# ArbiterMob/FluidSimulationCuda

Measured on AMD Instinct MI355X. Metric: Mcells/s per Jacobi iter, higher is better.
Workload: dtype f32

## Files before the change

### fluidsimulationcuda_amd/capi.py

```python
import ctypes as C
import os

import numpy as np

from ._build import LIB

OK, E_INVALID, E_NOMEM, E_HIP, E_COMM = 0, 1, 2, 3, 4
U, V, DENS, U_PREV, V_PREV, DENS_PREV, TMP0, TMP1, TMP2, TMP3, TMP4, TMP5 = range(12)
NFIELDS = 12
JACOBI_STREAM, JACOBI_LDS, JACOBI_NAIVE, JACOBI_TB = 0, 1, 2, 3
STORAGE_F32, STORAGE_F16 = 0, 1
PARAM_TB_MAX_SWEEPS, PARAM_TB_ROWS, PARAM_HALO, PARAM_TB_FAST_DIVISION, PARAM_TB_MIN_CELLS, PARAM_TB_EDGE_ROWS_PCT = 0, 1, 2, 3, 4, 5
PARAM_TB_LANE_COLUMNS = 6
PARAM_TB_T16_MIN_CELLS = 7
PARAM_TB_AUTOTUNE = 8
PARAM_FUSE_DIVERGENCE = 9
PARAM_SLAB_OVERLAP = 10
PARAM_EARLY_ADVECT = 11
PARAM_FUSE_ADD_SOURCE = 12
PARAM_XCHG_OVERLAP = 13
PARAM_F16_PRESSURE_SCALE = 14
PARAM_TB_FILL = 15
XCHG_HALO, XCHG_GATHER, XCHG_MAX, XCHG_MAX_BEGIN, XCHG_MAX_END = 0, 1, 2, 3, 4
RCCL_ID_BYTES = 128
FIELD_NAMES = ("u", "v", "dens", "u_prev", "v_prev", "dens_prev", "tmp0", "tmp1", "tmp2", "tmp3", "tmp4", "tmp5")


class FluidError(RuntimeError):
    def __init__(self, code, msg):
        super().__init__("libfluid_amd error %d: %s" % (code, msg))
        self.code = code


class Config(C.Structure):
    _fields_ = [("n", C.c_int), ("rank", C.c_int), ("nranks", C.c_int), ("halo", C.c_int),
                ("jacobi_variant", C.c_int), ("stream", C.c_void_p), ("arena", C.c_void_p),
                ("arena_bytes", C.c_size_t), ("storage", C.c_int)]


TIME_SOURCE, TIME_DIFFUSION, TIME_DIVERGENCE, TIME_PROJECTION, TIME_ADVECTION = range(5)
TIMING_CATEGORIES = ("source", "diffusion", "divergence", "projection", "advection")


class Timing(C.Structure):
    _fields_ = [("jacobi_ms", C.c_double), ("sweeps", C.c_longlong), ("solves", C.c_longlong),
# ... 133 lines not shown
```

### fluidsimulationcuda_amd/csrc/fluid_ctx.h

```cpp
#pragma once
#include <hip/hip_runtime.h>

#include <string>
#include <utility>
#include <vector>

#include "../../include/fluid_amd.h"
#include "fluid_kernels.h"

namespace fluid_detail {
int fail(int code, const char* fmt, ...);
int materialize_zero(fluid_ctx* c, int f);
int refuse_ensemble(const fluid_ctx* c, const char* what);
struct RcclExchange;
void rccl_release(RcclExchange* x);
}

#define HIP_TRY(expr)                                                                                      \
    do {                                                                                                   \
        hipError_t e_ = (expr);                                                                            \
        if (e_ != hipSuccess)                                                                              \
            return fluid_detail::fail(e_ == hipErrorOutOfMemory ? FLUID_E_NOMEM : FLUID_E_HIP, "%s: %s",   \
                                      #expr, hipGetErrorString(e_));                                       \
    } while (0)
// ... 88 lines not shown
    hipEvent_t ev_xbegin = nullptr, ev_xdone = nullptr;
    bool xchg_overlap = true;
    unsigned xowed = 0;
    long long split_launches = 0;
    bool early_advect = true;
    float vmax_prev[2] = {-1.0f, -1.0f};
    FieldState field[FLUID_NFIELDS];
    size_t field_bytes = 0;
    unsigned int* d_scalar = nullptr;
    float* d_partials = nullptr;
    ConstRing consts;
    EnsembleReduce red;
    MemberStage stage;
    TransformTables xform;
    unsigned int* tiles = nullptr;
    unsigned int* h_scalar = nullptr;
    hipEvent_t scalar_ready = nullptr;
    int variant = fluid::JACOBI_TB;
    int tb_max_t = 16, tb_rows = 0, num_cu = 256;
    long long tb_min_cells = 0;
    long long tb_t16_min_cells = -1;
    bool fuse_divergence = true;
    bool tb_fill = true;
    bool autotune = true;
    struct Trial { unsigned long long key; int cand; hipEvent_t a, b; };
    std::vector<Trial> trials;
    std::vector<hipEvent_t> free_events;
    bool defer_zero_source = true;
    bool in_halo_exchange = false;
    int tb_nv = 2;
    int tb_edge_pct = 40;
    int fast_div = 2;
    int rank = 0, nranks = 1, own0 = 1, own1 = 1, min_slab = 0, halo = 1;
    bool fuse_add_source = true;
    float pscale = 1.0f;
    fluid_exchange_fn xchg = nullptr;
    void* xchg_user = nullptr;
    fluid_detail::RcclExchange* rccl = nullptr;
    bool timing = false;
    struct Ev { hipEvent_t a, b; int cat; bool pressure; };
    std::vector<Ev> ev_pool;
    size_t ev_used = 0;
    double cat_ms[FLUID_TIMING_CATEGORIES] = {};
    long long cat_calls[FLUID_TIMING_CATEGORIES] = {};
    long long sweeps = 0, pending_sweeps = 0, launches = 0, field_launches = 0;
    double pressure_ms = 0.0;
// ... 13 lines not shown
```

### fluidsimulationcuda_amd/csrc/fluid_kernels.h

```cpp
#pragma once
#include <hip/hip_runtime.h>

namespace fluid {

constexpr int XOFF = 63;

enum JacobiVariant { JACOBI_STREAM = 0, JACOBI_LDS = 1, JACOBI_NAIVE = 2, JACOBI_TB = 3, JACOBI_VARIANTS = 4 };

enum Storage { STORAGE_F32 = 0, STORAGE_F16 = 1 };
typedef _Float16 half_t;
inline size_t storage_bytes(int st) { return st == STORAGE_F16 ? 2 : 4; }

inline int pitch_for(int n) { return ((XOFF + 1 + 4 * ((n + 3) / 4) + 1) + 63) / 64 * 64; }

struct Members {
    int count = 1;
    size_t stride = 0;
};

struct TbMemberK {
    double yd;
    float alpha, beta, hi, lo;
    float x0_inc, div_scale;
    unsigned tile_thr, pad;
};

struct TbBatch {
    const void* x[3];
    const void* x0[3];
    void* out[3];
    float alpha[3], beta[3];
    double yd[3];
    float hi[3], lo[3];
    const unsigned* tiles[3];
    unsigned tile_thr[3];
    int tile_pitch;
    void* div[3];
    float div_scale;
    int b[3];
    int x_zero[3];
    float x0_inc[3];
    int count;
    int members;
    size_t mstride;
    size_t tile_mstride;
    const TbMemberK* mk;
};

void launch_set_bnd(hipStream_t s, int st, void* f, int pitch, int n, int b, Members mb = {});
void launch_add_source(hipStream_t s, int st, void* x, const void* src, int pitch, int row_lo, int row_hi, float dt, Members mb = {},
                       const float* mdt = nullptr);
void launch_jacobi(hipStream_t s, int st, int variant, const void* x, const void* x0, void* out, int pitch, int n,
                   int row_lo, int row_hi, float alpha, float beta, int b, Members mb = {}, const float2* mab = nullptr);
enum TbForm { TB_PLAIN = 0, TB_DIVSRC = 1, TB_ADDSRC = 2 };
struct TbShape { int T, divmode, nv, form; };
inline constexpr TbShape kTbShapes[] = {
    {2, 0, 2, TB_PLAIN},   {2, 2, 2, TB_PLAIN},   {2, 3, 2, TB_PLAIN},   {2, 4, 2, TB_PLAIN},   {2, 5, 2, TB_PLAIN},
    {2, 0, 4, TB_PLAIN},   {2, 2, 4, TB_PLAIN},   {2, 3, 4, TB_PLAIN},   {2, 4, 4, TB_PLAIN},   {2, 5, 4, TB_PLAIN},
    {4, 0, 2, TB_PLAIN},   {4, 2, 2, TB_PLAIN},   {4, 3, 2, TB_PLAIN},   {4, 4, 2, TB_PLAIN},   {4, 5, 2, TB_PLAIN},
    {4, 0, 4, TB_PLAIN},   {4, 2, 4, TB_PLAIN},   {4, 3, 4, TB_PLAIN},   {4, 4, 4, TB_PLAIN},   {4, 5, 4, TB_PLAIN},
    {8, 0, 2, TB_PLAIN},   {8, 2, 2, TB_PLAIN},   {8, 3, 2, TB_PLAIN},   {8, 4, 2, TB_PLAIN},   {8, 5, 2, TB_PLAIN},
    {8, 0, 4, TB_PLAIN},   {8, 2, 4, TB_PLAIN},   {8, 3, 4, TB_PLAIN},   {8, 4, 4, TB_PLAIN},   {8, 5, 4, TB_PLAIN},
    {12, 0, 2, TB_PLAIN},  {12, 2, 2, TB_PLAIN},  {12, 3, 2, TB_PLAIN},  {12, 4, 2, TB_PLAIN},  {12, 5, 2, TB_PLAIN},
// ... 77 lines not shown
```

### fluidsimulationcuda_amd/csrc/fluid_kernels.hip

```cpp
#include <hip/hip_runtime.h>
#include <stdint.h>

#include <algorithm>
#include <array>
#include <cstdlib>
#include <utility>

#include "fluid_kernels.h"

namespace fluid {

__device__ __forceinline__ float flip_if(bool c, float v) { return c ? -v : v; }

__device__ __forceinline__ float keep_f32(float v) { asm("" : "+v"(v)); return v; }
__device__ __forceinline__ float ld1(const float* p) { return *p; }
__device__ __forceinline__ float ld1(const half_t* p) { return keep_f32((float)*p); }
__device__ __forceinline__ void st1(float* p, float v) { *p = v; }
__device__ __forceinline__ void st1(half_t* p, float v) { *p = (half_t)keep_f32(v); }
template <typename S>
__device__ __forceinline__ float as_stored(float v)
{
    if constexpr (sizeof(S) == 2) return keep_f32((float)(S)keep_f32(v));
    else return v;
}
// ... 376 lines not shown
constexpr float kDiv5NegScale = -0x1p24f;

template <typename S, int NV>
struct TbArgs {
    const S* xc;
    const S* rc;
    S* oc;
    __amdgpu_buffer_rsrc_t bx, br, bo;
    unsigned ld_off;
    unsigned st_off;
    unsigned row_bytes;
    unsigned m_lg;
    unsigned m_r[NV];
    int n, q_lo, q_hi, cg;
    float alpha;
    DivK k;
    S* dc;
    __amdgpu_buffer_rsrc_t bd;
    float div_scale;
    int s_lo, s_hi;
    unsigned sx, sy;
    float x0_inc;
    bool st_rg_lane, is_lg;
    bool fill;
};

__device__ __forceinline__ float fxor(float v, unsigned m) { return __uint_as_float(__float_as_uint(v) ^ m); }
template <int NV>
__device__ __forceinline__ Vec<NV> fxorv(const Vec<NV>& v, unsigned m)
{
    Vec<NV> o;
#pragma unroll
    for (int c = 0; c < NV; ++c) o.c[c] = fxor(v.c[c], m);
    return o;
}

template <int DIVMODE>
__device__ __forceinline__ float tb_div(float num, const DivK& k)
{
    if (DIVMODE == 0) return num / k.beta;
    if (DIVMODE == 4) return num * k.beta;
    if (DIVMODE == 3) return __builtin_fmaf(num, k.hi, num * k.lo);
    if (DIVMODE == 5) {
        const float q0 = num * k.beta;
        const float e = __builtin_fmaf(q0, k.hi, num * kDiv5NegScale);
        return __builtin_fmaf(e, k.lo, q0);
// ... 44 lines not shown
{
    unsigned long long n = 0;
    const unsigned long long stride = (unsigned long long)gridDim.x * 256;
    auto differs = [](float got, float ref) { return (ref != ref) ? !(got != got) : (__float_as_uint(got) != __float_as_uint(ref)); };
    DivK k2 = k;
    for (unsigned long long i = (unsigned long long)blockIdx.x * 256 + threadIdx.x; i < (1ull << 32); i += stride) {
        const float a = __uint_as_float((unsigned)i);
        const float ref = a / beta;
        if constexpr (DIVMODE == 3) {
            const bool in_range = a == 0.0f || !(__builtin_fabsf(a) < beta * 0x1p-98f);
            n += differs(tb_div<2>(a, k2), ref) || (in_range && differs(tb_div<3>(a, k), ref));
        } else if constexpr (DIVMODE == 5) {
            const float got = tb_div<5>(a, k);
            const bool finite = __builtin_fabsf(got) < __builtin_inff();
            const bool must_be_exact = __builtin_fabsf(a) < 0x1p100f;
            n += differs(got, ref) && (finite || must_be_exact);
        } else {
            n += differs(tb_div<DIVMODE>(a, k), ref);
        }
    }
    if (n) atomicAdd(bad, n);
}

__device__ __forceinline__ float bitsel(unsigned mask, float a, float b)
{
    return __uint_as_float((__float_as_uint(a) & mask) | (__float_as_uint(b) & ~mask));
}

template <typename S, int NV>
__device__ __forceinline__ void tb_fix_columns(Vec<NV>& G, const TbArgs<S, NV>& a, float& v1, float& vn, bool need_corners)
{
    float o[NV];
#pragma unroll
    for (int c = 0; c < NV; ++c) o[c] = G.c[c];
    const float from_right = lane_above0(o[0]);
    const float from_left = lane_below0(o[NV - 1]);
    G.c[0] = bitsel(a.m_r[0], fxor(from_left, a.sx), o[0]);
#pragma unroll
    for (int c = 1; c < NV - 1; ++c) G.c[c] = bitsel(a.m_r[c], fxor(o[c - 1], a.sx), o[c]);
    G.c[NV - 1] = bitsel(a.m_lg, fxor(from_right, a.sx), bitsel(a.m_r[NV - 1], fxor(o[NV - 2], a.sx), o[NV - 1]));
    if (need_corners) {
        v1 = from_right;
        unsigned bits = __float_as_uint(from_left) & a.m_r[0];
#pragma unroll
        for (int c = 1; c < NV; ++c) bits |= __float_as_uint(o[c - 1]) & a.m_r[c];
        vn = __uint_as_float(bits);
    }
}

template <bool EDGE, bool WALL, typename S, int NV>
__device__ __forceinline__ void tb_store_to(S* oc, __amdgpu_buffer_rsrc_t bo, const Vec<NV>& G, int q, bool mine, const TbArgs<S, NV>& a,
                                            float v1, float vn)
{
    auto on = [](bool c, unsigned off) { return c ? off : kBufOff; };
    buf_stv<NV>(oc, bo, on(mine, a.st_off) + (unsigned)q * a.row_bytes, G);
    if (WALL) {
        Vec<NV> g = fxorv<NV>(G, a.sy);
        if (EDGE) {
            const float cl = 0.5f * (fxor(v1, a.sy) + fxor(v1, a.sx));
            const float cr = 0.5f * (fxor(vn, a.sy) + fxor(vn, a.sx));
            if (a.is_lg) g.c[NV - 1] = cl;
#pragma unroll
            for (int c = 0; c < NV; ++c)
                if (a.st_rg_lane && a.cg == c) g.c[c] = cr;
        }
        buf_stv<NV>(oc, bo, on(mine & (q == 1), a.st_off), g);
        buf_stv<NV>(oc, bo, on(mine & (q == a.n), a.st_off) + (unsigned)(a.n + 1) * a.row_bytes, g);
    }
}
template <bool EDGE, bool WALL, typename S, int NV>
__device__ __forceinline__ void tb_store(const Vec<NV>& G, int q, bool mine, const TbArgs<S, NV>& a, float v1, float vn)
{
    tb_store_to<EDGE, WALL, S, NV>(a.oc, a.bo, G, q, mine, a, v1, vn);
}

template <int NV>
__device__ __forceinline__ Vec<NV> tb_divergence(const Vec<NV>& u, const Vec<NV>& v_up, const Vec<NV>& v_dn, float scale)
{
    float g[NV];
#pragma unroll
    for (int c = 0; c < NV; ++c) {
        const float ur = c < NV - 1 ? u.c[c + 1] : lane_above0(u.c[0]);
        const float ul = c > 0 ? u.c[c - 1] : lane_below0(u.c[NV - 1]);
        g[c] = ur - ul;
    }
    Vec<NV> d;
#pragma unroll
    for (int p = 0; p < NV; p += 2) {
        v2f s = {g[p], g[p + 1]};
        s = s + (v2f){v_dn.c[p], v_dn.c[p + 1]};
        s = s - (v2f){v_up.c[p], v_up.c[p + 1]};
        s = s * scale;
        d.c[p] = s.x;
// ... 14 lines not shown
        o.c[p + 1] = out.y;
    }
    return o;
}

template <int K, int N, int NV>
__device__ __forceinline__ void tb_qshift(Vec<NV> (&Q)[N])
{
    if constexpr (K >= 1) {
        Q[K] = Q[K - 1];
        tb_qshift<K - 1, N, NV>(Q);
    }
}

template <int DIVMODE, int NV>
__device__ __forceinline__ void tb_sticky(const Vec<NV>& G, v2f& nf)
{
    if constexpr (DIVMODE == 5) {
#pragma unroll
        for (int p = 0; p < NV; p += 2) nf = __builtin_elementwise_fma((v2f){G.c[p], G.c[p + 1]}, (v2f){0.f, 0.f}, nf);
    }
}

template <int T, int DIVMODE, bool EDGE, bool WALL, bool GEN, int PH, typename S, int NV, bool DIVSRC = false, bool ADDSRC = false,
          bool PART = false>
__device__ __forceinline__ void tb_step(int t, Vec<NV> (&W)[T][3], Vec<NV> (&Q)[T + 1], Vec<NV> (&PX)[3], Vec<NV> (&PQ)[3],
                                        const TbArgs<S, NV>& a, Vec<NV> (&UR)[3], Vec<NV> (&VR)[3], v2f& nf, int smax = T)
{
    static_assert(!(PART && GEN), "the general body runs every stage");
    constexpr int UP = PH % 3, ME = (PH + 1) % 3, FR = (PH + 2) % 3;
    __builtin_amdgcn_sched_barrier(0);
    if constexpr (DIVSRC) {
        UR[FR] = take<NV>(PX[PH]);
        VR[FR] = take<NV>(PQ[PH]);
    } else {
        W[0][FR] = take<NV>(PX[PH]);
        Q[0] = take<NV>(PQ[PH]);
        if constexpr (ADDSRC) {
#pragma unroll
            for (int p = 0; p < NV; p += 2) {
                const v2f ds = (v2f){W[0][FR].c[p], W[0][FR].c[p + 1]} * a.div_scale;
                const v2f q = (v2f){Q[0].c[p], Q[0].c[p + 1]} + ds;
                Q[0].c[p] = as_stored<S>(q.x);
                Q[0].c[p + 1] = as_stored<S>(q.y);
            }
            buf_stv<NV>(a.dc, a.bd, (((t >= a.s_lo) & (t < a.s_hi)) ? a.st_off : kBufOff) + (unsigned)t * a.row_bytes, Q[0]);
        } else {
#pragma unroll
            for (int p = 0; p < NV; p += 2) {
                const v2f q = (v2f){Q[0].c[p], Q[0].c[p + 1]} + a.x0_inc;
                Q[0].c[p] = q.x;
                Q[0].c[p + 1] = q.y;
            }
        }
    }
    {
        const unsigned off = a.ld_off + (unsigned)(t + 3) * a.row_bytes;
        PX[PH] = buf_ldv<NV>(a.xc, a.bx, off);
        PQ[PH] = buf_ldv<NV>(a.rc, a.br, off);
    }
    __builtin_amdgcn_sched_barrier(0);
    if constexpr (DIVSRC) {
        const int q = t - 1;
        Vec<NV> D = tb_divergence<NV>(UR[ME], VR[UP], VR[FR], a.div_scale);
#pragma unroll
        for (int c = 0; c < NV; ++c) D.c[c] = as_stored<S>(D.c[c]);
        Q[1] = D;
        float v1 = 0.f, vn = 0.f;
        if (EDGE) tb_fix_columns<S, NV>(D, a, v1, vn, WALL);
        tb_store_to<EDGE, (WALL || GEN), S, NV>(a.dc, a.bd, D, q, (q >= 1) & (q <= a.n) & (q >= a.q_lo) & (q < a.q_hi), a, v1, vn);
    }
    if constexpr (!GEN) {
#pragma unroll
        for (int s = 1; s <= T; ++s) {
            const bool run = !PART || s <= smax;
            const int q = t - s;
            Vec<NV> G;
            float v1 = 0.f, vn = 0.f;
            if (run) {
                G = tb_stencil<DIVMODE, NV>(W[s - 1][UP], W[s - 1][ME], W[s - 1][FR], Q[s], a.alpha, a.k);
                if (EDGE) tb_fix_columns<S, NV>(G, a, v1, vn, WALL && s == T);
                if (s == T) tb_sticky<DIVMODE, NV>(G, nf);
            } else {
#pragma unroll
                for (int c = 0; c < NV; ++c) G.c[c] = __builtin_nondeterministic_value(W[s - 1][FR].c[c]);
            }
            if (s < T) W[s][FR] = G;
            else tb_store<EDGE, WALL, S, NV>(G, q, run & (q >= a.q_lo) & (q < a.q_hi), a, v1, vn);
        }
    } else {
#pragma unroll
        for (int s = 1; s <= T; ++s) {
            const int q = t - s;
            const bool interior = (q >= 1 && q <= a.n);
            Vec<NV> G = tb_stencil<DIVMODE, NV>(W[s - 1][UP], W[s - 1][ME], W[s - 1][FR], Q[s], a.alpha, a.k);
            float v1 = 0.f, vn = 0.f;
            if (EDGE) tb_fix_columns<S, NV>(G, a, v1, vn, s == T);
            if (s < T) {
                const Vec<NV> me = W[s][ME];
                const Vec<NV> flipped_me = fxorv<NV>(me, a.sy);
                const Vec<NV> flipped_g = fxorv<NV>(G, a.sy);
                const bool bot_ghost = (q == a.n + 1), top_ghost = (q == 1);
#pragma unroll
                for (int c = 0; c < NV; ++c) {
                    W[s][FR].c[c] = bot_ghost ? flipped_me.c[c] : G.c[c];
                    W[s][ME].c[c] = top_ghost ? flipped_g.c[c] : me.c[c];
                }
            } else {
                tb_sticky<DIVMODE, NV>(G, nf);
                tb_store<EDGE, true, S, NV>(G, q, interior & (q >= a.q_lo) & (q < a.q_hi), a, v1, vn);
            }
        }
    }
    tb_qshift<T, T + 1, NV>(Q);
}

template <int T, int DIVMODE, bool EDGE, bool WALL, typename S, int NV, bool DIVSRC = false, bool ADDSRC = false>
__device__ __forceinline__ bool tb_march(int t0, int t1, const TbArgs<S, NV>& a)
{
    Vec<NV> W[T][3], Q[T + 1], PX[3], PQ[3], UR[3], VR[3];
    v2f nf = {0.f, 0.f};
    Vec<NV> zero;
#pragma unroll
    for (int c = 0; c < NV; ++c) zero.c[c] = 0.f;
#pragma unroll
    for (int s = 0; s < T; ++s) { W[s][0] = zero; W[s][1] = zero; W[s][2] = zero; }
#pragma unroll
    for (int s = 0; s <= T; ++s) Q[s] = zero;
#pragma unroll
    for (int d = 0; d < 3; ++d) { UR[d] = zero; VR[d] = zero; }
#pragma unroll
    for (int d = 0; d < 3; ++d) {
        const unsigned off = a.ld_off + (unsigned)(t0 + d) * a.row_bytes;
        PX[d] = buf_ldv<NV>(a.xc, a.bx, off);
        PQ[d] = buf_ldv<NV>(a.rc, a.br, off);
        buf_stv<NV>(a.oc, a.bo, kBufOff, zero);
        if constexpr (DIVSRC || ADDSRC) buf_stv<NV>(a.dc, a.bd, kBufOff, zero);
        __builtin_amdgcn_sched_barrier(0);
    }
    int t = t0;
// ... 13 lines not shown
        tb_step<T, DIVMODE, EDGE, WALL, false, 2, S, NV, DIVSRC, ADDSRC, true>(t + 2, W, Q, PX, PQ, a, UR, VR, nf, stages(t + 2));
    }
    for (; t <= full_end && (!WALL || t + 1 <= a.n); t += 3) {
        tb_step<T, DIVMODE, EDGE, WALL, false, 0, S, NV, DIVSRC, ADDSRC>(t, W, Q, PX, PQ, a, UR, VR, nf);
        tb_step<T, DIVMODE, EDGE, WALL, false, 1, S, NV, DIVSRC, ADDSRC>(t + 1, W, Q, PX, PQ, a, UR, VR, nf);
        tb_step<T, DIVMODE, EDGE, WALL, false, 2, S, NV, DIVSRC, ADDSRC>(t + 2, W, Q, PX, PQ, a, UR, VR, nf);
    }
    for (; t <= t1 && (!WALL || t + 1 <= a.n); t += 3) {
        tb_step<T, DIVMODE, EDGE, WALL, false, 0, S, NV, DIVSRC, ADDSRC, true>(t, W, Q, PX, PQ, a, UR, VR, nf, stages(t));
        tb_step<T, DIVMODE, EDGE, WALL, false, 1, S, NV, DIVSRC, ADDSRC, true>(t + 1, W, Q, PX, PQ, a, UR, VR, nf, stages(t + 1));
        tb_step<T, DIVMODE, EDGE, WALL, false, 2, S, NV, DIVSRC, ADDSRC, true>(t + 2, W, Q, PX, PQ, a, UR, VR, nf, stages(t + 2));
    }
    if constexpr (WALL) {
        for (; t <= t1; t += 3) {
            tb_step<T, DIVMODE, EDGE, WALL, true, 0, S, NV, DIVSRC, ADDSRC>(t, W, Q, PX, PQ, a, UR, VR, nf);
            tb_step<T, DIVMODE, EDGE, WALL, true, 1, S, NV, DIVSRC, ADDSRC>(t + 1, W, Q, PX, PQ, a, UR, VR, nf);
            tb_step<T, DIVMODE, EDGE, WALL, true, 2, S, NV, DIVSRC, ADDSRC>(t + 2, W, Q, PX, PQ, a, UR, VR, nf);
        }
    }
    if constexpr (DIVMODE == 5) return __builtin_amdgcn_ballot_w64((nf.x != nf.x) | (nf.y != nf.y)) != 0ull;
    else return false;
}

template <int T, int DIVMODE, typename S, int NV, bool DIVSRC = false, bool ADDSRC = false>
__device__ __forceinline__ bool tb_march_any(bool edge, bool wall, int t0, int t1, const TbArgs<S, NV>& a)
{
    if (edge) {
        if (wall) return tb_march<T, DIVMODE, true, true, S, NV, DIVSRC, ADDSRC>(t0, t1, a);
        return tb_march<T, DIVMODE, true, false, S, NV, DIVSRC, ADDSRC>(t0, t1, a);
    }
    if (wall) return tb_march<T, DIVMODE, false, true, S, NV, DIVSRC, ADDSRC>(t0, t1, a);
    return tb_march<T, DIVMODE, false, false, S, NV, DIVSRC, ADDSRC>(t0, t1, a);
}

struct TbGrid {
    int inner_wins, inner_blocks, edge_wins, edge_blocks, first_right;
    int hole_lo, hole_hi;
};

constexpr int tb_waves_per_simd(int T, int NV) { return NV == 2 ? (T <= 8 ? 4 : T <= 12 ? 3 : 2) : (T <= 4 ? 3 : 2); }

template <int T, int DIVMODE, int NV, typename S, bool DIVSRC = false, bool ADDSRC = false>
__global__ __launch_bounds__(256, tb_waves_per_simd(T, NV)) void k_jacobi_tb(TbBatch batch, int pitch, int n, int row_lo,
                                                                             int row_hi, int rb, int rb_edge, TbGrid g, int fill)
{
    static_assert(!DIVSRC || DIVMODE == 4, "the divergence-sourced launch is the first launch of a pressure solve");
    static_assert(!(DIVSRC && ADDSRC) && (!ADDSRC || DIVMODE != 3), "one second store per launch; mode 3's tiles are taken from the summed field");
    const unsigned per_xcd = gridDim.x >> 3;
    unsigned vid = (blockIdx.x & 7u) * per_xcd + (blockIdx.x >> 3);
    if (vid >= (unsigned)(g.inner_blocks + g.edge_blocks)) return;
    int win, strip_group;
    if (vid < (unsigned)g.inner_blocks) {
        win = 1 + (int)(vid % (unsigned)g.inner_wins);
        strip_group = (int)(vid / (unsigned)g.inner_wins);
    } else {
// ... 15 lines not shown
    if (batch.mk != nullptr) {
        typedef const TbMemberK __attribute__((address_space(4))) * MemberKPtr;
        const MemberKPtr mk = (MemberKPtr)(uintptr_t)batch.mk + ((size_t)sv * (unsigned)batch.members + member);
        alpha = mk->alpha;
        beta = mk->beta;
        yd = mk->yd;
        k_hi = mk->hi;
        k_lo = mk->lo;
        x0_inc = mk->x0_inc;
        if (ADDSRC) div_scale = mk->div_scale;
        if (DIVMODE == 3) tile_thr = mk->tile_thr;
    }
    const int b = batch.b[sv];
    constexpr int HL = (T + NV - 1) / NV;
    constexpr int VS = 64 - 2 * HL;
    constexpr int C0 = (XOFF + 1) / NV;
    static_assert((XOFF + 1) % NV == 0 && HL <= C0, "window overlap must fit the row's left pad");
    const int lane = threadIdx.x & 63;
    const int strip = strip_group * 4 + __builtin_amdgcn_readfirstlane(threadIdx.x >> 6);
    const int kg = n / NV;
    const bool left_edge = (win == 0);
    const bool right_edge = (kg >= win * VS - HL) && (kg < win * VS - HL + 64);
    const bool edge = left_edge || right_edge;
    const int rbw = edge ? rb_edge : rb;
    TbArgs<S, NV> a;
    a.k.yd = yd;
    a.k.lo = k_lo;
    a.k.hi = k_hi;
    a.x0_inc = x0_inc;
    int seg_hi = row_hi;
    a.q_lo = row_lo + strip * rbw;
    if (g.hole_lo < g.hole_hi) {
        const int top = (g.hole_lo - row_lo + rbw - 1) / rbw;
        if (strip < top) seg_hi = g.hole_lo;
        else a.q_lo = g.hole_hi + (strip - top) * rbw;
    }
    if (a.q_lo >= seg_hi) return;
    a.q_hi = min(a.q_lo + rbw, seg_hi);
    a.s_lo = a.q_lo == 1 ? 0 : a.q_lo;
    a.s_hi = a.q_hi == n + 1 ? n + 2 : a.q_hi;
    const int k = win * VS - HL + lane;
    const int nvec = (n + NV - 1) / NV;
    const bool ld_ok = k <= pitch / NV - C0 - 1;
    const ptrdiff_t cofs = (ptrdiff_t)(XOFF + 1) + NV * (ptrdiff_t)(ld_ok ? k : 0);
    a.xc = x + cofs;
    a.rc = x0 + cofs;
    a.oc = out + cofs;
    {
        const unsigned field_bytes = (unsigned)((size_t)(n + 2) * (size_t)pitch * sizeof(S));
        a.bx = __builtin_amdgcn_make_buffer_rsrc(const_cast<S*>(x), 0, (batch.x_zero[sv] && !DIVSRC) ? 0u : field_bytes, 0x00020000);
        a.br = __builtin_amdgcn_make_buffer_rsrc(const_cast<S*>(x0), 0, field_bytes, 0x00020000);
        a.bo = __builtin_amdgcn_make_buffer_rsrc(out, 0, field_bytes, 0x00020000);
        S* dv = (DIVSRC || ADDSRC) ? static_cast<S*>(batch.div[sv]) + mofs : out;
        a.dc = dv + cofs;
        a.bd = __builtin_amdgcn_make_buffer_rsrc(dv, 0, field_bytes, 0x00020000);
        a.div_scale = div_scale;
        a.row_bytes = (unsigned)((size_t)pitch * sizeof(S));
        const unsigned col = (unsigned)((XOFF + 1 + NV * (ptrdiff_t)k) * (ptrdiff_t)sizeof(S));
        a.ld_off = ld_ok ? col : kBufOff;
    }
    a.n = n;
    a.cg = n % NV;
    a.is_lg = (k == -1);
    const bool is_rg = (k == kg);
    const bool own = (lane >= HL) && (lane < 64 - HL);
    const bool st_int = own && k >= 0 && k < nvec;
    a.st_rg_lane = is_rg && (own || k == nvec);
    a.m_lg = a.is_lg ? 0xFFFFFFFFu : 0u;
#pragma unroll
    for (int c = 0; c < NV; ++c) a.m_r[c] = (is_rg && a.cg == c) ? 0xFFFFFFFFu : 0u;
    a.st_off = (ld_ok && (st_int || a.is_lg || a.st_rg_lane)) ? a.ld_off : kBufOff;
    a.sx = (b == 1) ? 0x80000000u : 0u;
    a.sy = (b == 2) ? 0x80000000u : 0u;
    a.alpha = alpha;
    a.k.beta = beta;
    a.fill = fill != 0;
    const int t0 = max(0, a.q_lo - T), t1 = a.q_hi - 1 + T;
    const bool wall = (a.q_lo < T) || (a.q_hi - 1 + T > n + 1);
    constexpr int DM = DIVMODE == 3 ? 2 : DIVMODE;
    bool two_term = false;
    if constexpr (DIVMODE == 3) {
        const unsigned* __restrict__ tiles = batch.tiles[sv] ? batch.tiles[sv] + (size_t)member * batch.tile_mstride : nullptr;
        const unsigned thr = tile_thr;
        const int tr0 = (max(1, a.q_lo - T + 1) - 1) / kTileRows, tr1 = (min(n, a.q_hi + T - 2) - 1) / kTileRows;
        const int c0 = max(1, 1 + NV * (win * VS - HL)), c1 = min(n, NV * (win * VS - HL + 64));
        const int tc0 = (c0 - 1) / kTileCols, tc1 = (c1 - 1) / kTileCols, ntc = tc1 - tc0 + 1;
        const int count = (tr1 - tr0 + 1) * ntc;
        bool low = false;
        if (tiles != nullptr)
            for (int i = lane; i < count; i += 64)
                low |= tiles[(size_t)(tr0 + i / ntc) * batch.tile_pitch + (tc0 + i % ntc)] < thr;
        two_term = tiles != nullptr && __builtin_amdgcn_ballot_w64(low) == 0ull;
    }
    if (two_term) {
        tb_march_any<T, DIVMODE, S, NV>(edge, wall, t0, t1, a);
    } else {
        const bool again = tb_march_any<T, DM, S, NV, DIVSRC, ADDSRC>(edge, wall, t0, t1, a);
        if constexpr (DIVMODE == 5) {
            if (again) tb_march_any<T, 2, S, NV, false, ADDSRC>(edge, wall, t0, t1, a);
        }
    }
}

template <typename S>
__global__ __launch_bounds__(256) void k_tile_min_abs(TileBatch tb, int pitch, int n, int row_lo, int row_hi, int tile_row0, int tile_pitch)
{
    const unsigned member = blockIdx.z / (unsigned)tb.count, sv = blockIdx.z - member * (unsigned)tb.count;
    const S* __restrict__ f = static_cast<const S*>(tb.field[sv]) + (size_t)member * tb.mstride;
    unsigned* __restrict__ out = tb.tiles[sv] + (size_t)member * tb.tile_mstride;
    const int lane = threadIdx.x & 63, wave = threadIdx.x >> 6;
    const int tr = tile_row0 + blockIdx.y;
    const int j = 1 + 4 * (lane + 64 * (blockIdx.x * 4 + wave));
    const int i0 = max(row_lo, 1 + tr * kTileRows), i1 = min(row_hi, 1 + (tr + 1) * kTileRows);
    const size_t P = (size_t)pitch;
    float m = __builtin_inff();
    if (j <= n)
        for (int i = i0; i < i1; ++i) {
            const float4 v = ld4(f + (size_t)i * P + XOFF + j);
            m = fminf(m, fabsf(v.x));
            if (j + 1 <= n) m = fminf(m, fabsf(v.y));
            if (j + 2 <= n) m = fminf(m, fabsf(v.z));
            if (j + 3 <= n) m = fminf(m, fabsf(v.w));
// ... 1198 lines not shown
```

### fluidsimulationcuda_amd/csrc/fluid_solver.hip

```cpp
#include <hip/hip_runtime.h>

#include <algorithm>
#include <cmath>
#include <cstdarg>
#include <cstdio>
#include <cstring>
#include <functional>
#include <mutex>
#include <new>
#include <string>
#include <unordered_map>
#include <vector>

#include "fluid_ctx.h"

namespace fluid_detail {

thread_local std::string g_err;

int fail(int code, const char* fmt, ...)
{
    char buf[512];
    va_list ap;
    va_start(ap, fmt);
// ... 465 lines not shown
        std::vector<int> cand;
        std::vector<float> best_ms;
        std::vector<int> samples, issued;
        int fixed = 0;
        std::string what;
    };
    std::mutex mu;
    std::unordered_map<unsigned long long, Entry> table;
};
RbTuner& rb_tuner()
{
    static RbTuner t;
    return t;
}
constexpr int kTuneSamples = 2;

unsigned long long tune_key(const fluid_ctx* c, int T, int m, int divmode, long long rows_n)
{
    int dev = 0;
    (void)hipGetDevice(&dev);
    unsigned long long h = 1469598103934665603ull;
    for (unsigned long long v : {(unsigned long long)dev, (unsigned long long)c->n, (unsigned long long)rows_n, (unsigned long long)T,
                                 (unsigned long long)m, (unsigned long long)divmode, (unsigned long long)c->tb_nv, (unsigned long long)c->st,
                                 (unsigned long long)c->tb_edge_pct, (unsigned long long)c->tb_fill,
                                 (unsigned long long)c->members}) {
        h ^= v;
        h *= 1099511628211ull;
    }
    return h;
}

void tune_harvest(fluid_ctx* c)
{
    if (c->trials.empty()) return;
    RbTuner& t = rb_tuner();
    std::lock_guard<std::mutex> lock(t.mu);
    size_t keep = 0;
    for (size_t k = 0; k < c->trials.size(); ++k) {
        fluid_ctx::Trial& tr = c->trials[k];
        if (hipEventQuery(tr.b) != hipSuccess) {
            c->trials[keep++] = tr;
            continue;
        }
        float ms = 0.f;
        auto it = t.table.find(tr.key);
        if (hipEventElapsedTime(&ms, tr.a, tr.b) == hipSuccess && it != t.table.end() && !it->second.fixed) {
            RbTuner::Entry& e = it->second;
// ... 273 lines not shown
    if (m == 0) return FLUID_OK;
    TRY(xchg_join(c));
    if (c->nranks > 1)
        HIP_TRY(hipMemsetAsync(solve_tiles(c, B.scratch_base), 0, (size_t)B.count * c->members * tile_words(c) * sizeof(unsigned), c->stream));
    int lo, hi;
    rows(c, std::min(valid, c->n), &lo, &hi);
    fluid::launch_tile_min_abs(c->stream, c->st, tb, m, c->pitch, c->n, lo, hi, fluid::tile_pitch(c->n), c->mb(), tile_words(c));
    return FLUID_OK;
}

int batch_reach(const fluid_ctx* c, const Batch& B)
{
    int r = kEverywhere;
    for (int k = 0; k < B.count; ++k) r = std::min(r, std::min(c->field[B.cur[k]].reach, c->field[B.sv[k].x0].reach + 1));
    return r;
}

fluid::TbMemberK solve_constants(const Batch& B, int j, int m, const MemberVal& x0_inc, const MemberVal& div_scale)
{
    const DivPlan& p = B.plan[j][B.plan[j].size() > 1 ? (size_t)m : 0];
    return {p.yd, B.sv[j].k->alpha.at(m), p.arg, p.hi, p.lo, x0_inc.at(m), div_scale.at(m), p.tile_thr, 0};
}

int fill_batch(fluid_ctx* c, const Batch& B, int first, int last, bool divsrc, bool addsrc, fluid::TbBatch* out)
{
    static const MemberVal nothing_pending(-0.0f);
    const MemberVal own_scale(divsrc ? B.ds->scale : 0.0f);
    const MemberVal& div_scale = addsrc ? c->field[B.sv[first].x0].src_dt : own_scale;
    const MemberVal* x0_inc[3];
    fluid::TbBatch bt{};
    bool per_member = !div_scale.uniform();
    for (int j = first; j < last; ++j) {
        const int q = j - first;
        const FieldState& x0 = c->field[B.sv[j].x0];
        x0_inc[q] = x0.pend && !addsrc && !divsrc ? &x0.pend_inc : &nothing_pending;
        per_member = per_member || B.plan[j].size() > 1 || !x0_inc[q]->uniform();
        const fluid::TbMemberK k0 = solve_constants(B, j, 0, *x0_inc[q], div_scale);
        bt.x[q] = c->ptr(B.cur[j]);
        bt.x0[q] = x0.ptr;
        bt.out[q] = c->ptr(B.nxt[j]);
        bt.alpha[q] = k0.alpha;
        bt.beta[q] = k0.beta;
        bt.yd[q] = k0.yd;
        bt.hi[q] = k0.hi;
        bt.lo[q] = k0.lo;
        bt.tiles[q] = B.plan[j][0].mode == 3 ? solve_tiles(c, B.scratch_base + j) : nullptr;
        bt.tile_thr[q] = k0.tile_thr;
        bt.b[q] = B.sv[j].b;
        bt.x_zero[q] = c->field[B.cur[j]].zero ? 1 : 0;
        bt.x0_inc[q] = k0.x0_inc;
        if (addsrc) bt.div[q] = c->ptr(B.sum[j]);
    }
    bt.count = last - first;
    bt.members = c->members;
    bt.mstride = c->field_floats;
    bt.tile_mstride = tile_words(c);
    bt.tile_pitch = fluid::tile_pitch(c->n);
    bt.div_scale = div_scale.at(0);
    if (divsrc) {
        bt.x[0] = c->ptr(B.ds->u);
        bt.x0[0] = c->ptr(B.ds->v);
        bt.div[0] = c->ptr(B.sv[0].x0);
    }
    if (per_member && c->members > 1) {
        const int M = c->members;
        std::vector<fluid::TbMemberK> rec((size_t)bt.count * M);
        for (int j = first; j < last; ++j)
            for (int m = 0; m < M; ++m) rec[(size_t)(j - first) * M + m] = solve_constants(B, j, m, *x0_inc[j - first], div_scale);
        const void* dev = nullptr;
        TRY(member_consts(c, rec.data(), rec.size() * sizeof rec[0], &dev));
        bt.mk = static_cast<const fluid::TbMemberK*>(dev);
    }
// ... 23 lines not shown
        const int low = std::max(2, std::min(rb, (int)(rows_n / 64) & ~1));
        if (c->members == 1 || fits(low)) rb = low;
        else rb = (int)std::min<long long>(rb, std::max<long long>(low, (rows_n + 1) & ~1ll));
    }
    return rb;
}

int launch_fused(fluid_ctx* c, const fluid::TbBatch& bt, int T, int divmode, bool divsrc, bool addsrc, int lo, int hi)
{
    const bool owed = c->nranks > 1 && (c->xowed & stream_bit(c));
    const int in_lo = owed && c->rank > 0 ? std::max(lo, c->own0 + T) : lo;
    const int in_hi = owed && c->rank < c->nranks - 1 ? std::min(hi, c->own1 - T) : hi;
    const bool split = owed && in_hi - in_lo >= 2 * T && (in_lo > lo || in_hi < hi);
    const int form = divsrc ? fluid::TB_DIVSRC : addsrc ? fluid::TB_ADDSRC : fluid::TB_PLAIN;
    for (int part = split ? 0 : 1; part < 2; ++part) {
        const int plo = part ? lo : in_lo, phi = part ? hi : in_hi;
        const int hole_lo = part && split ? in_lo : 0, hole_hi = part && split ? in_hi : 0;
        if (part) TRY(xchg_join(c));
        const long long rows_n = (phi - plo) - std::max(0, hole_hi - hole_lo);
        int rb = c->tb_rows > 0 ? c->tb_rows : strip_rows(c, T, bt.count * c->members, rows_n);
        int trial = -1;
        unsigned long long key = 0;
        if (c->tb_rows <= 0 && c->autotune) {
            key = tune_key(c, T, bt.count + (divsrc ? 8 : 0) + (addsrc ? 16 : 0) + (hole_hi > hole_lo ? 32 : 0), divmode, rows_n);
            rb = tune_pick(c, key, rb, T, rows_n, &trial, bt.count, form, divmode);
        }
        if (trial >= 0) TRY(tune_begin(c, key, trial));
        if (!fluid::launch_jacobi_tb(c->stream, c->st, T, divmode, c->tb_nv, form, bt, c->pitch, c->n, plo, phi, rb,
                                     std::min(rb, edge_rows(c, T, rb)), hole_lo, hole_hi, c->tb_fill))
            return fail(FLUID_E_INVALID, "no fused Jacobi kernel: %d sweeps, division mode %d, %d-column lanes, form %d", T, divmode, c->tb_nv, form);
        if (trial >= 0) TRY(tune_end(c));
    }
    if (split) c->split_launches += 1;
    return FLUID_OK;
}

void commit_launch(fluid_ctx* c, Batch& B, bool first, int r)
{
    if (B.ds && first && c->nranks > 1)
        c->field[B.sv[0].x0].reach = std::max(0, std::min(c->field[B.sv[0].x0].reach, r));
    if (B.add_src && first) {
        for (int j = 0; j < B.count; ++j) {
            trade(c, B.sv[j].x0, B.sum[j]);
            wrote(c, B.sum[j], 0);
            wrote(c, B.sv[j].x0, std::max(0, r));
        }
        B.add_src = false;
    }
    for (int j = 0; j < B.count; ++j) {
        c->field[B.cur[j]].zero = false;
        wrote(c, B.nxt[j], r);
        std::swap(B.cur[j], B.nxt[j]);
    }
}

int batch_sweep(fluid_ctx* c, Batch& B)
{
    const Solve* sv = B.sv;
    const bool multi = c->nranks > 1, canonical = B.shape.canonical;
    int r = multi ? batch_reach(c, B) : kEverywhere;
    for (int k = 0; k < B.iters;) {
        const int remaining = B.iters - k;
        const int wantT = canonical ? pick_sweeps(c, remaining, remaining, B.shape, B.all_mode4) : 1;
        if (r < wantT) {
            const int depth = std::max(wantT, std::min(c->halo, remaining + B.final_reach));
            std::vector<int> ids;
            for (int j = 0; j < B.count; ++j) {
                ids.push_back(B.cur[j]);
                if (c->field[sv[j].x0].reach < depth - 1) ids.push_back(sv[j].x0);
            }
            TRY(xchg_join(c));
            TRY(need_list(c, ids, depth, true));
            r = batch_reach(c, B);
        }
        const int T = canonical ? wantT : pick_sweeps(c, remaining, std::min(r, remaining), B.shape, B.all_mode4);
        if (B.add_src && k == 0 && !fluid::jacobi_tb_exists(T, B.plan[0][0].mode, c->tb_nv, fluid::TB_ADDSRC)) {
            B.add_src = false;
            TRY(xchg_join(c));
            for (int j = 0; j < B.count; ++j) TRY(settle_source(c, sv[j].x0));
        }
        int lo, hi;
        rows(c, multi ? std::min(r - T, exchange_cap(c)) : 0, &lo, &hi);
        if (T == 1) {
            const int v = c->variant == fluid::JACOBI_TB ? (B.shape.small ? fluid::JACOBI_NAIVE : fluid::JACOBI_STREAM) : c->variant;
            TRY(xchg_join(c));
            for (int j = 0; j < B.count; ++j) TRY(materialize(c, B.cur[j], true));
            for (int j = 0; j < B.count; ++j) TRY(settle(c, sv[j].x0, true));
            for (int j = 0; j < B.count; ++j) {
                const float2* mab = nullptr;
                TRY(member_pairs(c, sv[j].k->alpha, sv[j].k->beta, &mab));
                fluid::launch_jacobi(c->stream, c->st, v, c->ptr(B.cur[j]), c->ptr(sv[j].x0), c->ptr(B.nxt[j]), c->pitch, c->n, lo, hi,
                                     sv[j].k->alpha.at(0), sv[j].k->beta.at(0), sv[j].b, c->mb(), mab);
            }
            if (c->timing) {
                c->launches += B.count;
                c->field_launches += (long long)B.count * c->members;
            }
        } else {
            for (int first = 0, last; first < B.count; first = last) {
                last = B.same_mode ? B.count : first + 1;
                const bool divsrc = B.ds != nullptr && k == 0, addsrc = B.add_src && k == 0;
                fluid::TbBatch bt;
                TRY(fill_batch(c, B, first, last, divsrc, addsrc, &bt));
                TRY(launch_fused(c, bt, T, B.plan[first][0].mode, divsrc, addsrc, lo, hi));
                if (c->timing) {
                    c->launches += 1;
                    c->field_launches += (long long)(last - first) * c->members;
                }
            }
        }
        r = multi ? std::min(r - T, exchange_cap(c)) : kEverywhere;
        commit_launch(c, B, k == 0, r);
        k += T;
    }
    return FLUID_OK;
}

int op_diffuse_batch(fluid_ctx* c, const Solve* sv, int count, int iters, int final_reach = 0, const DivSource* ds = nullptr,
                     int scratch_base = 0)
{
    Batch B{sv, count, iters, final_reach, ds, scratch_base};
    TRY(batch_prepare(c, B));
    if (iters == 0) return FLUID_OK;
    hipEvent_t stop;
    TRY(timing_begin(c, FLUID_TIME_DIFFUSION, &stop));
    TRY(batch_plan(c, B));
    TRY(batch_sweep(c, B));
    HIP_TRY(hipGetLastError());
    for (int j = 0; j < count; ++j) {
        if (B.cur[j] != sv[j].x) trade(c, sv[j].x, B.scratch[j]);
        wrote(c, B.scratch[j], 0);
        c->field[sv[j].x].fscale = B.out_scale[j];
    }
    return timing_end(c, stop, iters * count * c->members);
// ... 718 lines not shown
        return FLUID_OK;
    case FLUID_PARAM_TB_ROWS:
        if (value < 0) return fail(FLUID_E_INVALID, "TB_ROWS must be >= 0");
        c->tb_rows = value;
        return FLUID_OK;
    case FLUID_PARAM_TB_EDGE_ROWS_PCT:
        if (value < 0 || value > 100) return fail(FLUID_E_INVALID, "TB_EDGE_ROWS_PCT must be in [0,100]");
        c->tb_edge_pct = value;
        return FLUID_OK;
    case FLUID_PARAM_TB_MIN_CELLS:
        if (value < 0) return fail(FLUID_E_INVALID, "TB_MIN_CELLS must be >= 0");
        c->tb_min_cells = value;
        return FLUID_OK;
    case FLUID_PARAM_TB_FAST_DIVISION:
        if (value < 0 || value > 3) return fail(FLUID_E_INVALID, "TB_FAST_DIVISION must be 0, 1, 2 or 3");
        c->fast_div = value;
        return FLUID_OK;
    case FLUID_PARAM_TB_AUTOTUNE:
        c->autotune = value != 0;
        return FLUID_OK;
    case FLUID_PARAM_TB_FILL:
        c->tb_fill = value != 0;
        return FLUID_OK;
    case FLUID_PARAM_SLAB_OVERLAP:
        c->slab_overlap = value != 0;
        return FLUID_OK;
    case FLUID_PARAM_FUSE_DIVERGENCE:
        c->fuse_divergence = value != 0;
        return FLUID_OK;
    case FLUID_PARAM_EARLY_ADVECT:
        c->early_advect = value != 0;
        return FLUID_OK;
    case FLUID_PARAM_FUSE_ADD_SOURCE:
        c->fuse_add_source = value != 0;
        return FLUID_OK;
    case FLUID_PARAM_F16_PRESSURE_SCALE: {
        for (int f = 0; f < FLUID_NFIELDS; ++f) TRY(unscale(c, f));
        int e = 0;
        (void)std::frexp((float)c->n, &e);
        c->pscale = (value != 0 && c->st == fluid::STORAGE_F16 && c->n >= 16) ? std::ldexp(1.0f, e - 3) : 1.0f;
        return FLUID_OK;
    }
    case FLUID_PARAM_XCHG_OVERLAP:
        TRY(xchg_join(c));
        c->xchg_overlap = value != 0;
        return FLUID_OK;
// ... 1034 lines not shown
```

### include/fluid_amd.h

```cpp
#ifndef FLUID_AMD_H
#define FLUID_AMD_H

#include <stddef.h>

#ifdef __cplusplus
extern "C" {
#endif

#define FLUID_OK        0
#define FLUID_E_INVALID 1
#define FLUID_E_NOMEM   2
#define FLUID_E_HIP     3
#define FLUID_E_COMM    4

enum {
    FLUID_U = 0, FLUID_V = 1, FLUID_DENS = 2,
    FLUID_U_PREV = 3, FLUID_V_PREV = 4, FLUID_DENS_PREV = 5,
    FLUID_TMP0 = 6, FLUID_TMP1 = 7, FLUID_TMP2 = 8,
    FLUID_TMP3 = 9, FLUID_TMP4 = 10, FLUID_TMP5 = 11,
    FLUID_NFIELDS = 12
};

enum { FLUID_JACOBI_STREAM = 0, FLUID_JACOBI_LDS = 1, FLUID_JACOBI_NAIVE = 2, FLUID_JACOBI_TB = 3 };

enum {
    FLUID_PARAM_TB_MAX_SWEEPS = 0,
    FLUID_PARAM_TB_ROWS = 1,
    FLUID_PARAM_HALO = 2,
    FLUID_PARAM_TB_FAST_DIVISION = 3
    ,FLUID_PARAM_TB_EDGE_ROWS_PCT = 5
    ,FLUID_PARAM_TB_LANE_COLUMNS = 6
    ,FLUID_PARAM_TB_T16_MIN_CELLS = 7
    ,FLUID_PARAM_TB_AUTOTUNE = 8
    ,FLUID_PARAM_SLAB_OVERLAP = 10
    ,FLUID_PARAM_EARLY_ADVECT = 11
    ,FLUID_PARAM_FUSE_DIVERGENCE = 9
    ,FLUID_PARAM_FUSE_ADD_SOURCE = 12
    ,FLUID_PARAM_XCHG_OVERLAP = 13
    ,FLUID_PARAM_F16_PRESSURE_SCALE = 14
    ,FLUID_PARAM_TB_FILL = 15
    ,FLUID_PARAM_TB_MIN_CELLS = 4
};

typedef struct fluid_ctx fluid_ctx;

const char *fluid_last_error(void);

int step(int N, float dt, float diff, float visc, float *u, float *v, float *dens);
int step_src(int N, float dt, float diff, float visc, int iters,
             float *u, float *v, float *dens,
             float *u_prev, float *v_prev, float *dens_prev);
int fluid_release_cached(void);

int fluid_coefficients(int N, float dt, float coef, float *alpha, float *beta);

typedef struct fluid_config {
    int n;
    int rank, nranks;
    int halo;
    int jacobi_variant;
    void *stream;
    void *arena;
    size_t arena_bytes;
// ... 145 lines not shown
```

Measured before the change: 4.286 million.

## Mirror edge-column images in temporal-blocked Jacobi instead of replaying boundary fixes

Adds a mirror edge mode for the temporally blocked Jacobi kernel. For fields whose boundary is a reflection (b=0 or 2), edge lanes load mirrored image columns and swap the lane pair, so the per-stage boundary column fix runs only on the final stage. Edge windows can then use the normal row-block size instead of the smaller edge-row count. The mode is on by default, only for NV=2 without fused divergence or add-source, and it adds a tuning-key bit. The risk is correctness at corners and extra load-address logic on edge wavefronts.

```diff
diff --git a/fluidsimulationcuda_amd/capi.py b/fluidsimulationcuda_amd/capi.py
--- a/fluidsimulationcuda_amd/capi.py
+++ b/fluidsimulationcuda_amd/capi.py
@@ -21,6 +21,7 @@
 PARAM_XCHG_OVERLAP = 13
 PARAM_F16_PRESSURE_SCALE = 14
 PARAM_TB_FILL = 15
+PARAM_TB_MIRROR = 16
 XCHG_HALO, XCHG_GATHER, XCHG_MAX, XCHG_MAX_BEGIN, XCHG_MAX_END = 0, 1, 2, 3, 4
 RCCL_ID_BYTES = 128
 FIELD_NAMES = ("u", "v", "dens", "u_prev", "v_prev", "dens_prev", "tmp0", "tmp1", "tmp2", "tmp3", "tmp4", "tmp5")
diff --git a/fluidsimulationcuda_amd/csrc/fluid_ctx.h b/fluidsimulationcuda_amd/csrc/fluid_ctx.h
--- a/fluidsimulationcuda_amd/csrc/fluid_ctx.h
+++ b/fluidsimulationcuda_amd/csrc/fluid_ctx.h
@@ -134,6 +134,7 @@
     long long tb_t16_min_cells = -1;
     bool fuse_divergence = true;
     bool tb_fill = true;
+    bool tb_mirror = true;
     bool autotune = true;
     struct Trial { unsigned long long key; int cand; hipEvent_t a, b; };
     std::vector<Trial> trials;
diff --git a/fluidsimulationcuda_amd/csrc/fluid_kernels.h b/fluidsimulationcuda_amd/csrc/fluid_kernels.h
--- a/fluidsimulationcuda_amd/csrc/fluid_kernels.h
+++ b/fluidsimulationcuda_amd/csrc/fluid_kernels.h
@@ -39,6 +39,7 @@
     float div_scale;
     int b[3];
     int x_zero[3];
+    int mirror[3];
     float x0_inc[3];
     int count;
     int members;
diff --git a/fluidsimulationcuda_amd/csrc/fluid_kernels.hip b/fluidsimulationcuda_amd/csrc/fluid_kernels.hip
--- a/fluidsimulationcuda_amd/csrc/fluid_kernels.hip
+++ b/fluidsimulationcuda_amd/csrc/fluid_kernels.hip
@@ -422,6 +422,7 @@
     unsigned sx, sy;
     float x0_inc;
     bool st_rg_lane, is_lg;
+    unsigned sw0, sw1;
     bool fill;
 };
 
@@ -512,9 +513,20 @@
     if (n) atomicAdd(bad, n);
 }
 
+constexpr int TB_EDGE_NONE = 0, TB_EDGE_REPLAY = 1, TB_EDGE_MIRROR = 2;
+
 __device__ __forceinline__ float bitsel(unsigned mask, float a, float b)
 {
     return __uint_as_float((__float_as_uint(a) & mask) | (__float_as_uint(b) & ~mask));
+}
+
+template <typename S, int NV>
+__device__ __forceinline__ void tb_image(Vec<NV>& v, const TbArgs<S, NV>& a)
+{
+    static_assert(NV == 2, "a lane's image is its pair reversed");
+    const float c0 = v.c[0], c1 = v.c[1];
+    v.c[0] = bitsel(a.sw0, c1, c0);
+    v.c[1] = bitsel(a.sw1, c0, c1);
 }
 
 template <typename S, int NV>
@@ -538,7 +550,7 @@
     }
 }
 
-template <bool EDGE, bool WALL, typename S, int NV>
+template <int EDGE, bool WALL, typename S, int NV>
 __device__ __forceinline__ void tb_store_to(S* oc, __amdgpu_buffer_rsrc_t bo, const Vec<NV>& G, int q, bool mine, const TbArgs<S, NV>& a,
                                             float v1, float vn)
 {
@@ -558,7 +570,7 @@
         buf_stv<NV>(oc, bo, on(mine & (q == a.n), a.st_off) + (unsigned)(a.n + 1) * a.row_bytes, g);
     }
 }
-template <bool EDGE, bool WALL, typename S, int NV>
+template <int EDGE, bool WALL, typename S, int NV>
 __device__ __forceinline__ void tb_store(const Vec<NV>& G, int q, bool mine, const TbArgs<S, NV>& a, float v1, float vn)
 {
     tb_store_to<EDGE, WALL, S, NV>(a.oc, a.bo, G, q, mine, a, v1, vn);
@@ -619,12 +631,13 @@
     }
 }
 
-template <int T, int DIVMODE, bool EDGE, bool WALL, bool GEN, int PH, typename S, int NV, bool DIVSRC = false, bool ADDSRC = false,
+template <int T, int DIVMODE, int EDGE, bool WALL, bool GEN, int PH, typename S, int NV, bool DIVSRC = false, bool ADDSRC = false,
           bool PART = false>
 __device__ __forceinline__ void tb_step(int t, Vec<NV> (&W)[T][3], Vec<NV> (&Q)[T + 1], Vec<NV> (&PX)[3], Vec<NV> (&PQ)[3],
                                         const TbArgs<S, NV>& a, Vec<NV> (&UR)[3], Vec<NV> (&VR)[3], v2f& nf, int smax = T)
 {
     static_assert(!(PART && GEN), "the general body runs every stage");
+    static_assert(EDGE != TB_EDGE_MIRROR || !(DIVSRC || ADDSRC), "the launches that form their right-hand side replay set_bnd");
     constexpr int UP = PH % 3, ME = (PH + 1) % 3, FR = (PH + 2) % 3;
     __builtin_amdgcn_sched_barrier(0);
     if constexpr (DIVSRC) {
@@ -633,6 +646,10 @@
     } else {
         W[0][FR] = take<NV>(PX[PH]);
         Q[0] = take<NV>(PQ[PH]);
+        if constexpr (EDGE == TB_EDGE_MIRROR) {
+            tb_image<S, NV>(W[0][FR], a);
+            tb_image<S, NV>(Q[0], a);
+        }
         if constexpr (ADDSRC) {
 #pragma unroll
             for (int p = 0; p < NV; p += 2) {
@@ -676,7 +693,7 @@
             float v1 = 0.f, vn = 0.f;
             if (run) {
                 G = tb_stencil<DIVMODE, NV>(W[s - 1][UP], W[s - 1][ME], W[s - 1][FR], Q[s], a.alpha, a.k);
-                if (EDGE) tb_fix_columns<S, NV>(G, a, v1, vn, WALL && s == T);
+                if (EDGE == TB_EDGE_REPLAY || (EDGE == TB_EDGE_MIRROR && s == T)) tb_fix_columns<S, NV>(G, a, v1, vn, WALL && s == T);
                 if (s == T) tb_sticky<DIVMODE, NV>(G, nf);
             } else {
 #pragma unroll
@@ -692,7 +709,7 @@
             const bool interior = (q >= 1 && q <= a.n);
             Vec<NV> G = tb_stencil<DIVMODE, NV>(W[s - 1][UP], W[s - 1][ME], W[s - 1][FR], Q[s], a.alpha, a.k);
             float v1 = 0.f, vn = 0.f;
-            if (EDGE) tb_fix_columns<S, NV>(G, a, v1, vn, s == T);
+            if (EDGE == TB_EDGE_REPLAY || (EDGE == TB_EDGE_MIRROR && s == T)) tb_fix_columns<S, NV>(G, a, v1, vn, s == T);
             if (s < T) {
                 const Vec<NV> me = W[s][ME];
                 const Vec<NV> flipped_me = fxorv<NV>(me, a.sy);
@@ -712,7 +729,7 @@
     tb_qshift<T, T + 1, NV>(Q);
 }
 
-template <int T, int DIVMODE, bool EDGE, bool WALL, typename S, int NV, bool DIVSRC = false, bool ADDSRC = false>
+template <int T, int DIVMODE, int EDGE, bool WALL, typename S, int NV, bool DIVSRC = false, bool ADDSRC = false>
 __device__ __forceinline__ bool tb_march(int t0, int t1, const TbArgs<S, NV>& a)
 {
     Vec<NV> W[T][3], Q[T + 1], PX[3], PQ[3], UR[3], VR[3];
@@ -772,15 +789,23 @@
     else return false;
 }
 
+template <int NV, bool DIVSRC, bool ADDSRC>
+constexpr bool tb_mirror_form = NV == 2 && !DIVSRC && !ADDSRC;
 template <int T, int DIVMODE, typename S, int NV, bool DIVSRC = false, bool ADDSRC = false>
-__device__ __forceinline__ bool tb_march_any(bool edge, bool wall, int t0, int t1, const TbArgs<S, NV>& a)
+__device__ __forceinline__ bool tb_march_any(bool edge, bool mirror, bool wall, int t0, int t1, const TbArgs<S, NV>& a)
 {
     if (edge) {
-        if (wall) return tb_march<T, DIVMODE, true, true, S, NV, DIVSRC, ADDSRC>(t0, t1, a);
-        return tb_march<T, DIVMODE, true, false, S, NV, DIVSRC, ADDSRC>(t0, t1, a);
-    }
-    if (wall) return tb_march<T, DIVMODE, false, true, S, NV, DIVSRC, ADDSRC>(t0, t1, a);
-    return tb_march<T, DIVMODE, false, false, S, NV, DIVSRC, ADDSRC>(t0, t1, a);
+        if constexpr (tb_mirror_form<NV, DIVSRC, ADDSRC>) {
+            if (mirror) {
+                if (wall) return tb_march<T, DIVMODE, TB_EDGE_MIRROR, true, S, NV>(t0, t1, a);
+                return tb_march<T, DIVMODE, TB_EDGE_MIRROR, false, S, NV>(t0, t1, a);
+            }
+        }
+        if (wall) return tb_march<T, DIVMODE, TB_EDGE_REPLAY, true, S, NV, DIVSRC, ADDSRC>(t0, t1, a);
+        return tb_march<T, DIVMODE, TB_EDGE_REPLAY, false, S, NV, DIVSRC, ADDSRC>(t0, t1, a);
+    }
+    if (wall) return tb_march<T, DIVMODE, TB_EDGE_NONE, true, S, NV, DIVSRC, ADDSRC>(t0, t1, a);
+    return tb_march<T, DIVMODE, TB_EDGE_NONE, false, S, NV, DIVSRC, ADDSRC>(t0, t1, a);
 }
 
 struct TbGrid {
@@ -842,7 +867,8 @@
     const bool left_edge = (win == 0);
     const bool right_edge = (kg >= win * VS - HL) && (kg < win * VS - HL + 64);
     const bool edge = left_edge || right_edge;
-    const int rbw = edge ? rb_edge : rb;
+    const bool mirror = tb_mirror_form<NV, DIVSRC, ADDSRC> && batch.mirror[sv] != 0;
+    const int rbw = (edge && !mirror) ? rb_edge : rb;
     TbArgs<S, NV> a;
     a.k.yd = yd;
     a.k.lo = k_lo;
@@ -886,10 +912,25 @@
     const bool own = (lane >= HL) && (lane < 64 - HL);
     const bool st_int = own && k >= 0 && k < nvec;
     a.st_rg_lane = is_rg && (own || k == nvec);
+    if (mirror) a.st_rg_lane = is_rg && (own || (k == nvec && lane == 64 - HL));
     a.m_lg = a.is_lg ? 0xFFFFFFFFu : 0u;
 #pragma unroll
     for (int c = 0; c < NV; ++c) a.m_r[c] = (is_rg && a.cg == c) ? 0xFFFFFFFFu : 0u;
     a.st_off = (ld_ok && (st_int || a.is_lg || a.st_rg_lane)) ? a.ld_off : kBufOff;
+    a.sw0 = a.sw1 = 0u;
+    if constexpr (tb_mirror_form<NV, DIVSRC, ADDSRC>) {
+        if (edge && mirror) {
+            const bool left_img = k < 0, right_img = k > kg - (a.cg == 0 ? 1 : 0);
+            const int ki = left_img ? -1 - k : 2 * kg - 1 + a.cg - k;
+            if (left_img || right_img) {
+                const bool reach = (left_img || k - kg <= HL) && ki >= 0 && ki <= kg;
+                a.ld_off = reach ? (unsigned)((XOFF + 1 + NV * (ptrdiff_t)ki) * (ptrdiff_t)sizeof(S)) : kBufOff;
+                a.sw0 = a.sw1 = 0xFFFFFFFFu;
+            } else if (is_rg) {
+                a.sw1 = 0xFFFFFFFFu;
+            }
+        }
+    }
     a.sx = (b == 1) ? 0x80000000u : 0u;
     a.sy = (b == 2) ? 0x80000000u : 0u;
     a.alpha = alpha;
@@ -913,11 +954,11 @@
         two_term = tiles != nullptr && __builtin_amdgcn_ballot_w64(low) == 0ull;
     }
     if (two_term) {
-        tb_march_any<T, DIVMODE, S, NV>(edge, wall, t0, t1, a);
+        tb_march_any<T, DIVMODE, S, NV>(edge, mirror, wall, t0, t1, a);
     } else {
-        const bool again = tb_march_any<T, DM, S, NV, DIVSRC, ADDSRC>(edge, wall, t0, t1, a);
+        const bool again = tb_march_any<T, DM, S, NV, DIVSRC, ADDSRC>(edge, mirror, wall, t0, t1, a);
         if constexpr (DIVMODE == 5) {
-            if (again) tb_march_any<T, 2, S, NV, false, ADDSRC>(edge, wall, t0, t1, a);
+            if (again) tb_march_any<T, 2, S, NV, false, ADDSRC>(edge, mirror, wall, t0, t1, a);
         }
     }
 }
diff --git a/fluidsimulationcuda_amd/csrc/fluid_solver.hip b/fluidsimulationcuda_amd/csrc/fluid_solver.hip
--- a/fluidsimulationcuda_amd/csrc/fluid_solver.hip
+++ b/fluidsimulationcuda_amd/csrc/fluid_solver.hip
@@ -511,7 +511,7 @@
     unsigned long long h = 1469598103934665603ull;
     for (unsigned long long v : {(unsigned long long)dev, (unsigned long long)c->n, (unsigned long long)rows_n, (unsigned long long)T,
                                  (unsigned long long)m, (unsigned long long)divmode, (unsigned long long)c->tb_nv, (unsigned long long)c->st,
-                                 (unsigned long long)c->tb_edge_pct, (unsigned long long)c->tb_fill,
+                                 (unsigned long long)c->tb_edge_pct, (unsigned long long)c->tb_fill, (unsigned long long)c->tb_mirror,
                                  (unsigned long long)c->members}) {
         h ^= v;
         h *= 1099511628211ull;
@@ -831,7 +831,7 @@
     return {p.yd, B.sv[j].k->alpha.at(m), p.arg, p.hi, p.lo, x0_inc.at(m), div_scale.at(m), p.tile_thr, 0};
 }
 
-int fill_batch(fluid_ctx* c, const Batch& B, int first, int last, bool divsrc, bool addsrc, fluid::TbBatch* out)
+int fill_batch(fluid_ctx* c, const Batch& B, int first, int last, bool divsrc, bool addsrc, int T, bool fused_before, fluid::TbBatch* out)
 {
     static const MemberVal nothing_pending(-0.0f);
     const MemberVal own_scale(divsrc ? B.ds->scale : 0.0f);
@@ -857,6 +857,8 @@
         bt.tile_thr[q] = k0.tile_thr;
         bt.b[q] = B.sv[j].b;
         bt.x_zero[q] = c->field[B.cur[j]].zero ? 1 : 0;
+        bt.mirror[q] = c->tb_mirror && c->tb_nv == 2 && !divsrc && !addsrc && (B.sv[j].b == 0 || B.sv[j].b == 2) && c->n >= 2 * T &&
+                       (bt.x_zero[q] || fused_before);
         bt.x0_inc[q] = k0.x0_inc;
         if (addsrc) bt.div[q] = c->ptr(B.sum[j]);
     }
@@ -926,7 +928,9 @@
         int trial = -1;
         unsigned long long key = 0;
         if (c->tb_rows <= 0 && c->autotune) {
-            key = tune_key(c, T, bt.count + (divsrc ? 8 : 0) + (addsrc ? 16 : 0) + (hole_hi > hole_lo ? 32 : 0), divmode, rows_n);
+            const bool mirrors = bt.mirror[0] || bt.mirror[1] || bt.mirror[2];
+            key = tune_key(c, T, bt.count + (divsrc ? 8 : 0) + (addsrc ? 16 : 0) + (hole_hi > hole_lo ? 32 : 0) + (mirrors ? 64 : 0), divmode,
+                           rows_n);
             rb = tune_pick(c, key, rb, T, rows_n, &trial, bt.count, form, divmode);
         }
         if (trial >= 0) TRY(tune_begin(c, key, trial));
@@ -963,6 +967,7 @@
     const Solve* sv = B.sv;
     const bool multi = c->nranks > 1, canonical = B.shape.canonical;
     int r = multi ? batch_reach(c, B) : kEverywhere;
+    bool fused_before = false;
     for (int k = 0; k < B.iters;) {
         const int remaining = B.iters - k;
         const int wantT = canonical ? pick_sweeps(c, remaining, remaining, B.shape, B.all_mode4) : 1;
@@ -1005,7 +1010,7 @@
                 last = B.same_mode ? B.count : first + 1;
                 const bool divsrc = B.ds != nullptr && k == 0, addsrc = B.add_src && k == 0;
                 fluid::TbBatch bt;
-                TRY(fill_batch(c, B, first, last, divsrc, addsrc, &bt));
+                TRY(fill_batch(c, B, first, last, divsrc, addsrc, T, fused_before, &bt));
                 TRY(launch_fused(c, bt, T, B.plan[first][0].mode, divsrc, addsrc, lo, hi));
                 if (c->timing) {
                     c->launches += 1;
@@ -1014,6 +1019,7 @@
             }
         }
         r = multi ? std::min(r - T, exchange_cap(c)) : kEverywhere;
+        fused_before = T > 1;
         commit_launch(c, B, k == 0, r);
         k += T;
     }
@@ -1778,6 +1784,9 @@
     case FLUID_PARAM_TB_FILL:
         c->tb_fill = value != 0;
         return FLUID_OK;
+    case FLUID_PARAM_TB_MIRROR:
+        c->tb_mirror = value != 0;
+        return FLUID_OK;
     case FLUID_PARAM_SLAB_OVERLAP:
         c->slab_overlap = value != 0;
         return FLUID_OK;
diff --git a/include/fluid_amd.h b/include/fluid_amd.h
--- a/include/fluid_amd.h
+++ b/include/fluid_amd.h
@@ -39,6 +39,7 @@
     ,FLUID_PARAM_XCHG_OVERLAP = 13
     ,FLUID_PARAM_F16_PRESSURE_SCALE = 14
     ,FLUID_PARAM_TB_FILL = 15
+    ,FLUID_PARAM_TB_MIRROR = 16
     ,FLUID_PARAM_TB_MIN_CELLS = 4
 };
 
```

Result: slower. 4.076 million (-4.9%).
